# Yixin-F/DR-Using-SCV-OD

Measured on AMD Instinct MI355X. Metric: scans/sec on SemanticKITTI-seq-05-shaped input (SCV-OD dynamic-removal path, raw scans -> per-point labels + static map), higher is better.
Workload: dtype f32

## Files before the change

### dr-using-scv-od_amd/csrc/scvod_k_patchwork.inc

```
constexpr int kClsThreads = 256;
constexpr int kClsItems = 8;

__global__ __launch_bounds__(kClsThreads) void k_pw_classify(DevParams P, Arena A) {
    __shared__ int hist[kMaxPatches];
    const int s = blockIdx.y;
    const int base = A.scan_off[s];
    const int n = A.scan_off[s + 1] - base;
    const int start = blockIdx.x * (kClsThreads * kClsItems);
    if (start >= n) return;
    for (int b = threadIdx.x; b < P.n_patches; b += kClsThreads) hist[b] = 0;
    __syncthreads();
    float4 pt[kClsItems];
#pragma unroll
    for (int it = 0; it < kClsItems; ++it) {
        const int i = start + it * kClsThreads + threadIdx.x;
        pt[it] = A.pts[base + min(i, n - 1)];
    }
#pragma unroll
    for (int it = 0; it < kClsItems; ++it) {
        const int i = start + it * kClsThreads + threadIdx.x;
        if (i < n) {
            const float4 p = pt[it];
            int pid = czm_patch_of(P.czm, p.x, p.y, p.z);
            A.pid[base + i] = (int16_t)pid;
            A.zkey[base + i] = float_sort_key(p.z);
            if (pid >= 0) atomicAdd(&hist[pid], 1);
        }
    }
    __syncthreads();
    for (int b = threadIdx.x; b < P.n_patches; b += kClsThreads) {
        int c = hist[b];
        if (c) atomicAdd(&A.patch_count[s * kMaxPatches + b], c);
    }
}

__global__ __launch_bounds__(1024) void k_pw_offsets(DevParams P, Arena A) {
    __shared__ int wsum[17];
    const int s = blockIdx.x;
    int c = (threadIdx.x < (unsigned)P.n_patches) ? A.patch_count[s * kMaxPatches + threadIdx.x] : 0;
    int total;
    int ex = block_excl_scan<1024>(c, total, wsum);
    if (threadIdx.x <= (unsigned)P.n_patches) A.patch_off[s * (kMaxPatches + 1) + threadIdx.x] = ex;
}

__global__ __launch_bounds__(kClsThreads) void k_pw_scatter(DevParams P, Arena A) {
    __shared__ int hist[kMaxPatches];
    const int s = blockIdx.y;
    const int base = A.scan_off[s];
    const int n = A.scan_off[s + 1] - base;
    const int start = blockIdx.x * (kClsThreads * kClsItems);
    if (start >= n) return;
    for (int b = threadIdx.x; b < P.n_patches; b += kClsThreads) hist[b] = 0;
    __syncthreads();
    int pid[kClsItems], rank[kClsItems];
    uint32_t zk[kClsItems];
#pragma unroll
    for (int it = 0; it < kClsItems; ++it) {
        const int i = start + it * kClsThreads + threadIdx.x;
        pid[it] = (i < n) ? (int)A.pid[base + i] : -1;
        zk[it] = A.zkey[base + min(i, n - 1)];
    }
#pragma unroll
    for (int it = 0; it < kClsItems; ++it)
        rank[it] = wave_bin_rank(hist, pid[it]);
    __syncthreads();
    for (int b = threadIdx.x; b < P.n_patches; b += kClsThreads) {
        int c = hist[b];
        if (c) hist[b] = A.patch_off[s * (kMaxPatches + 1) + b] + atomicAdd(&A.patch_cursor[s * kMaxPatches + b], c);
    }
    __syncthreads();
#pragma unroll
    for (int it = 0; it < kClsItems; ++it) {
        int i = start + it * kClsThreads + threadIdx.x;
        if (i < n && pid[it] >= 0) A.keys[(size_t)base + hist[pid[it]] + rank[it]] = pack_key(zk[it], (uint32_t)i);
    }
}

constexpr int kClassXS = 32, kClassM = 40, kClassM2 = 44, kClassL = 48;
#ifndef SCVOD_FIT_COOP_CLASS
#define SCVOD_FIT_COOP_CLASS 36
#endif
constexpr int kClassFitCoop = SCVOD_FIT_COOP_CLASS;

__device__ __forceinline__ void order_range(const int32_t* off, int c_lo, int c_hi, int& lo, int& hi) {
    lo = off[c_hi];
    hi = (c_lo == 0) ? off[64] : off[c_lo - 1];
}

constexpr bool pw_sort_padfree(int cap) { return SCVOD_SORT_PADFREE == 2 || (SCVOD_SORT_PADFREE == 1 && cap >= 2048); }

template <int CAP, int THREADS, int C_LO, int C_HI, int LGE>
__global__ __launch_bounds__(THREADS)
__attribute__((amdgpu_waves_per_eu(pw_sort_padfree(CAP) ? (CAP >= 1024 ? 4 : 6) : 1, 8)))
void k_pw_sort(DevParams P, Arena A) {
    extern __shared__ __attribute__((aligned(16))) unsigned char smem[];
    int lo, hi;
    order_range(A.order_off, C_LO, C_HI, lo, hi);
    constexpr int PK = (CAP == 4096) ? 1 : 2;
    constexpr bool PADFREE = pw_sort_padfree(CAP);
    PROF_BEGIN();
    for (int w = lo + blockIdx.x; w < hi; w += gridDim.x) {
        const int4 item = A.order[w];
        const int n = item.y, base = item.z, off = item.w;
        const bool in_lds = (n <= CAP);
        unsigned long long* keys;
        if (CAP >= 4096) PROF_RESET();
        if (in_lds) {
            keys = (unsigned long long*)smem;
            int np2 = 1 << LGE;
            while (np2 < n) np2 <<= 1;
            const int nlive = sortnet::live_end(n, LGE);
            constexpr int IT = CAP / THREADS;
            const unsigned long long* gk = (const unsigned long long*)A.keys + (size_t)base + off;
            bool from_regs = false;
            if constexpr (IT == (1 << LGE) && CAP >= 4096) {
                if (np2 == CAP) {
                    from_regs = true;
                    unsigned long long tmp[IT];
                    if constexpr (PADFREE) {
                        if ((int)threadIdx.x < (nlive >> LGE)) {
#pragma unroll
                            for (int it = 0; it < IT; ++it) {
                                const int j = sortnet::start_key(it, (int)threadIdx.x, nlive, LGE);
                                tmp[it] = (j < n) ? gk[j] : kKeyPad;
                            }
                        }
                        if (CAP >= 4096) PROF_MARK(PK, 0);
                        padfree_sort_regs<THREADS, true, LGE>(tmp, keys, np2, nlive, (unsigned long long)kKeyPad);
                    } else {
#pragma unroll
                        for (int it = 0; it < IT; ++it) {
                            const int j = it * THREADS + (int)threadIdx.x;
                            tmp[it] = (j < n) ? gk[j] : kKeyPad;
                        }
                        if (CAP >= 4096) PROF_MARK(PK, 0);
                        block_bitonic_sort_pow2_regs<THREADS, true, LGE>(tmp, keys);
                    }
                }
            }
            if (!from_regs) {
                const int nfill = PADFREE ? nlive : np2;
                for (int j = threadIdx.x; j < nfill; j += THREADS) keys[sort_slot<true>(j)] = (j < n) ? gk[j] : kKeyPad;
                __syncthreads();
                if (CAP >= 4096) PROF_MARK(PK, 0);
                if constexpr (PADFREE)
                    padfree_sort<THREADS, true, LGE>(keys, np2, nlive, (unsigned long long)kKeyPad);
                else
                    block_bitonic_sort_pow2<THREADS, true, LGE>(keys, np2);
            }
            if (CAP >= 4096) PROF_MARK(PK, 1);
        } else {
            keys = (unsigned long long*)(A.keys + (size_t)base + off);
            block_bitonic_sort<THREADS, false>(keys, n);
        }
        Xyz* dst = A.sorted_xyz + (size_t)base + off;
        uint32_t* dsti = A.sorted_idx + (size_t)base + off;
        for (int j0 = threadIdx.x; j0 < n; j0 += 4 * THREADS) {
            uint32_t id[4];
            float4 q[4];
#pragma unroll
            for (int u = 0; u < 4; ++u) {
                const int j = min(j0 + u * THREADS, n - 1);
                id[u] = key_idx(keys[in_lds ? sort_slot<true>(j) : j]);
            }
#pragma unroll
            for (int u = 0; u < 4; ++u) q[u] = A.pts[base + id[u]];
#pragma unroll
            for (int u = 0; u < 4; ++u) {
                const int j = j0 + u * THREADS;
                if (j < n) {
                    Xyz o;
                    o.x = q[u].x;
                    o.y = q[u].y;
                    o.z = q[u].z;
                    dst[j] = o;
                    dsti[j] = id[u];
                }
            }
        }
        __syncthreads();
        if (CAP >= 4096) PROF_MARK(PK, 2);
    }
}

constexpr int kClassWave = 24;
__global__ __launch_bounds__(256) void k_pw_sort_wave(DevParams P, Arena A) {
    const int lane = threadIdx.x & 63;
    const int wave = threadIdx.x >> 6;
    int lo, hi;
    order_range(A.order_off, 0, kClassWave - 1, lo, hi);
    for (int w = lo + blockIdx.x * 4 + wave; w < hi; w += gridDim.x * 4) {
        const int4 item = A.order[w];
        const int n = item.y, base = item.z, off = item.w;
        unsigned long long key = (lane < n) ? A.keys[(size_t)base + off + lane] : kKeyPad;
#pragma unroll
        for (int k = 2; k <= 64; k <<= 1) {
#pragma unroll
            for (int j = k >> 1; j >= 1; j >>= 1) {
                const unsigned long long other = __shfl_xor(key, j, 64);
                const bool take_min = (((lane & k) == 0) == ((lane & j) == 0));
                unsigned long long mn = key, mx = other;
                cswap_asc(mn, mx);
                key = take_min ? mn : mx;
            }
        }
        if (lane < n) {
            const uint32_t id = key_idx(key);
            const float4 q = A.pts[base + id];
            Xyz o;
            o.x = q.x;
            o.y = q.y;
            o.z = q.z;
            A.sorted_xyz[(size_t)base + off + lane] = o;
            A.sorted_idx[(size_t)base + off + lane] = id;
        }
    }
}

__device__ __forceinline__ int pw_size_class(int n) {
    int lg = 31 - __clz(n);
    int frac = (lg >= 2) ? ((n >> (lg - 2)) & 3) : 0;
    int c = lg * 4 + frac;
    return c > 63 ? 63 : c;
}

__global__ __launch_bounds__(256) void k_pw_order_count(DevParams P, Arena A) {
    __shared__ int hist[64];
    if (threadIdx.x < 64) hist[threadIdx.x] = 0;
    __syncthreads();
    const int t = blockIdx.x * 256 + threadIdx.x;
    if (t < A.n_scans * P.n_patches) {
        const int s = t / P.n_patches, p = t - s * P.n_patches;
        const int n = A.patch_count[s * kMaxPatches + p];
        if (n <= P.czm.num_min_pts) {
            PatchRec r = {n, 0, 0, 0, 0};
            A.patch_rec[s * kMaxPatches + p] = r;
            scvod_patch_plane pl = {};
            pl.n_pts = n;
            A.planes[s * kMaxPatches + p] = pl;
        } else {
            atomicAdd(&hist[pw_size_class(n)], 1);
        }
    }
    __syncthreads();
    if (threadIdx.x < 64 && hist[threadIdx.x]) atomicAdd(&A.order_hist[threadIdx.x], hist[threadIdx.x]);
}

__global__ __launch_bounds__(64) void k_pw_order_offsets(Arena A) {
    const int c = 63 - threadIdx.x;
    const int v = A.order_hist[c];
    const int inc = wave_incl_scan(v);
    A.order_off[c] = inc - v;
    if (threadIdx.x == 63) A.order_off[64] = inc;
}

__global__ __launch_bounds__(256) void k_pw_order_scatter(DevParams P, Arena A) {
    __shared__ int hist[64];
    if (threadIdx.x < 64) hist[threadIdx.x] = 0;
    __syncthreads();
    const int t = blockIdx.x * 256 + threadIdx.x;
    int c = -1, rank = 0;
    int4 item = make_int4(0, 0, 0, 0);
    if (t < A.n_scans * P.n_patches) {
        const int s = t / P.n_patches, p = t - s * P.n_patches;
        const int n = A.patch_count[s * kMaxPatches + p];
        if (n > P.czm.num_min_pts) {
            c = pw_size_class(n);
            rank = atomicAdd(&hist[c], 1);
            item = make_int4(s * kMaxPatches + p, n, A.scan_off[s], A.patch_off[s * (kMaxPatches + 1) + p]);
        }
    }
    __syncthreads();
    if (threadIdx.x < 64 && hist[threadIdx.x])
        hist[threadIdx.x] = A.order_off[threadIdx.x] + atomicAdd(&A.order_cursor[threadIdx.x], hist[threadIdx.x]);
    __syncthreads();
    if (c >= 0) A.order[hist[c] + rank] = item;
}

__global__ __launch_bounds__(256) void k_vx_order_count(DevParams P, Arena A) {
    __shared__ int hist[64];
    if (threadIdx.x < 64) hist[threadIdx.x] = 0;
    __syncthreads();
    const int t = blockIdx.x * 256 + threadIdx.x;
    if (t < A.n_scans * P.n_buckets) {
        const int s = t / P.n_buckets, b = t - s * P.n_buckets;
        const int m = A.vb_count[s * kMaxBuckets + b];
        if (m > 0)
            atomicAdd(&hist[pw_size_class(m)], 1);
        else
            A.vb_nvox[s * kMaxBuckets + b] = 0;
    }
    __syncthreads();
    if (threadIdx.x < 64 && hist[threadIdx.x]) atomicAdd(&A.vorder_hist[threadIdx.x], hist[threadIdx.x]);
}

__global__ __launch_bounds__(64) void k_vx_order_offsets(Arena A) {
    const int c = 63 - threadIdx.x;
    const int v = A.vorder_hist[c];
    const int inc = wave_incl_scan(v);
    A.vorder_off[c] = inc - v;
    if (threadIdx.x == 63) A.vorder_off[64] = inc;
}

__global__ __launch_bounds__(256) void k_vx_order_scatter(DevParams P, Arena A) {
    __shared__ int hist[64];
    if (threadIdx.x < 64) hist[threadIdx.x] = 0;
    __syncthreads();
    const int t = blockIdx.x * 256 + threadIdx.x;
    int c = -1, rank = 0;
    int4 item = make_int4(0, 0, 0, 0);
    if (t < A.n_scans * P.n_buckets) {
        const int s = t / P.n_buckets, b = t - s * P.n_buckets;
        const int m = A.vb_count[s * kMaxBuckets + b];
        if (m > 0) {
            c = pw_size_class(m);
            rank = atomicAdd(&hist[c], 1);
            item = make_int4(s * kMaxBuckets + b, m, A.scan_off[s], A.vb_off[s * (kMaxBuckets + 1) + b]);
        }
    }
    __syncthreads();
    if (threadIdx.x < 64 && hist[threadIdx.x])
        hist[threadIdx.x] = A.vorder_off[threadIdx.x] + atomicAdd(&A.vorder_cursor[threadIdx.x], hist[threadIdx.x]);
    __syncthreads();
    if (c >= 0) A.vorder[hist[c] + rank] = item;
}

__device__ __forceinline__ float plane_res(const Xyz& q, float n0, float n1, float n2) {
    float r = q.x * n0;
    r = r + q.y * n1;
    r = r + q.z * n2;
    return r;
}

struct FitState {
    float cov[9];
    float mean0, mean1, mean2;
    float n0, n1, n2, thd;
    float sv0, sv1, sv2;
};
__device__ __forceinline__ void fit_state_init(FitState& F) {
#pragma unroll
    for (int k = 0; k < 9; ++k) F.cov[k] = 0.f;
    F.mean0 = F.mean1 = F.mean2 = 0.f;
    F.n0 = F.n1 = F.n2 = F.thd = 0.f;
    F.sv0 = F.sv1 = F.sv2 = 0.f;
}

__device__ __forceinline__ void fit_update(FitState& F, const CzmParams& cz, float a0, float a1, float a2, float a3, float a4,
                                           float a5, float a6, float a7, float a8, int m) {
    if (m != 0) {
        const float fn = (float)m;
        a0 = a0 / fn;
        a1 = a1 / fn;
        a2 = a2 / fn;
        a3 = a3 / fn;
        a4 = a4 / fn;
        a5 = a5 / fn;
        a6 = a6 / fn;
        a7 = a7 / fn;
        a8 = a8 / fn;
        F.mean0 = a6;
        F.mean1 = a7;
        F.mean2 = a8;
        F.cov[0] = a0 - a6 * a6;
        F.cov[1] = a1 - a6 * a7;
        F.cov[2] = a2 - a6 * a8;
        F.cov[4] = a3 - a7 * a7;
        F.cov[5] = a4 - a7 * a8;
        F.cov[8] = a5 - a8 * a8;
        F.cov[3] = F.cov[1];
        F.cov[6] = F.cov[2];
        F.cov[7] = F.cov[5];
    }
    Svd3 sv;
    svd3_jacobi(F.cov, sv);
    F.n0 = sv.U[2];
    F.n1 = sv.U[5];
    F.n2 = sv.U[8];
    F.sv0 = sv.sv[0];
    F.sv1 = sv.sv[1];
    F.sv2 = sv.sv[2];
    float dot = F.n0 * F.mean0;
    dot = dot + F.n1 * F.mean1;
    dot = dot + F.n2 * F.mean2;
    const float d = -dot;
    F.thd = (float)(cz.th_dist - (double)d);
}

__device__ __forceinline__ int fit_status(const DevParams& P, int zone, int ring, int concentric_idx, const FitState& F) {
    const double ground_z_vec = (double)fabs_f(F.n2);
    const double ground_z_elevation = (double)F.mean2;
    float svmin = F.sv0;
    if (F.sv1 < svmin) svmin = F.sv1;
    if (F.sv2 < svmin) svmin = F.sv2;
    const double surface_variable = (double)(svmin / (F.sv0 + F.sv1 + F.sv2));
    if (ground_z_vec < P.czm.uprightness_thr) return 2;
    if (concentric_idx < P.czm.num_rings_of_interest) {
        const int e = ring + 2 * zone;
        if (ground_z_elevation > P.czm.elevation_thr[e]) return (P.czm.flatness_thr[e] > surface_variable) ? 1 : 3;
    }
    return 1;
}

__device__ __forceinline__ void fit_finish(const DevParams& P, const Arena& A, int s, int p, int n, int zone, int ring,
                                           int concentric_idx, const FitState& F) {
    const float n0 = F.n0, n1 = F.n1, n2 = F.n2, thd = F.thd, mean0 = F.mean0, mean1 = F.mean1, mean2 = F.mean2;
    const float sv0 = F.sv0, sv1 = F.sv1, sv2 = F.sv2;
    const int status = fit_status(P, zone, ring, concentric_idx, F);
    scvod_patch_plane pl;
    pl.normal[0] = n0;
    pl.normal[1] = n1;
    pl.normal[2] = n2;
    pl.mean[0] = mean0;
    pl.mean[1] = mean1;
    pl.mean[2] = mean2;
    pl.sv[0] = sv0;
    pl.sv[1] = sv1;
    pl.sv[2] = sv2;
    pl.n_pts = n;
    pl.n_ground = 0;
    pl.status = status;
    A.planes[s * kMaxPatches + p] = pl;
    A.fit_thd[s * kMaxPatches + p] = thd;
}

__device__ __forceinline__ uint32_t triple_of_point(const DevParams& P, float x, float y, float z) {
    int32_t ri, si, ai;
    if (!idx3_fast(P.bin, P.binfast, x, y, z, &ri, &si, &ai)) {
        Apri a;
        apri_of_point(P.bin, x, y, z, 0.f, a);
        ri = a.range_idx;
        si = a.sector_idx;
        ai = a.azimuth_idx;
    }
    return (uint32_t)pack_idx3(ri, si, ai);
}

template <int GL, bool LEAN>
__device__ __forceinline__ void arrange_group(const DevParams& P, const Arena& A, const Xyz* __restrict__ sp, const uint32_t* __restrict__ si, uint32_t* seg,
                                              uint32_t* stage, int n, int n_max, int slot, bool live, int r, int gbase, float n0, float n1, float n2, float thd, int status) {
    constexpr unsigned long long FULL = (GL == 64) ? ~0ull : ((1ull << (GL & 63)) - 1ull);
    auto group_bits = [&](unsigned long long ballot) -> unsigned long long { return (ballot >> gbase) & FULL; };
    const bool rejected = (status >= 2);
    const int n_last = max(n - 1, 0);
    int n_g = 0, n_ng = 0, a_g = 0, a_ng = 0;
    Xyz q_next = sp[min(r, n_last)];
    uint32_t w_next = si[min(r, n_last)];
    const unsigned long long below = (1ull << r) - 1ull;
// ... 706 lines not shown
```

### dr-using-scv-od_amd/csrc/scvod_kernels.hip

```cpp
#include <type_traits>

#include "scvod_boxgrid.h"
#include "scvod_grid.h"
#include "scvod_sortnet.h"
#include <rocprim/device/device_radix_sort.hpp>

namespace scvod {

#ifdef SCVOD_PROFILE
__device__ unsigned long long g_prof[8][16];
#define PROF_BEGIN() unsigned long long t_prev = wall_clock64()
#define PROF_RESET()                                   \
    do {                                               \
        __syncthreads();                               \
        if (threadIdx.x == 0) t_prev = wall_clock64(); \
    } while (0)
#define PROF_MARK(k, i)                                      \
    do {                                                     \
        __syncthreads();                                     \
        if (threadIdx.x == 0) {                              \
            const unsigned long long t_now = wall_clock64(); \
            atomicAdd(&g_prof[k][i], t_now - t_prev);        \
            t_prev = t_now;                                  \
        }                                                    \
    } while (0)
#else
#define PROF_BEGIN()
#define PROF_RESET()
#define PROF_MARK(k, i)
#endif
#define CC_MARK(i) PROF_MARK(0, i)
#define CCW_MARK(i) PROF_MARK(4, i)

template <typename T>
__device__ __forceinline__ void cswap(T& x, T& y) {
    const T lo = x < y ? x : y;
    const T hi = x < y ? y : x;
    x = lo;
    y = hi;
}

template <bool PAD>
__device__ __forceinline__ int sort_slot(int i) {
    return PAD ? i + (i >> 3) : i;
}

template <int THREADS, bool PAD, typename T>
__device__ __forceinline__ void block_bitonic_sort(T* a, int n) {
#define IX(i) sort_slot<PAD>(i)
    if (n <= 1) return;
    const T INF = ~(T)0;
    int np2 = 8;
    while (np2 < n) np2 <<= 1;
    for (int g = threadIdx.x; g < (np2 >> 3); g += THREADS) {
        const int b = g << 3;
        if (b >= n) continue;
        T e[8];
#pragma unroll
        for (int m = 0; m < 8; ++m) e[m] = (b + m < n) ? a[IX(b + m)] : INF;
        cswap(e[0], e[1]); cswap(e[2], e[3]); cswap(e[4], e[5]); cswap(e[6], e[7]);
        cswap(e[0], e[2]); cswap(e[1], e[3]); cswap(e[4], e[6]); cswap(e[5], e[7]);
        cswap(e[1], e[2]); cswap(e[5], e[6]);
        cswap(e[0], e[4]); cswap(e[1], e[5]); cswap(e[2], e[6]); cswap(e[3], e[7]);
        cswap(e[2], e[4]); cswap(e[3], e[5]);
        cswap(e[1], e[2]); cswap(e[3], e[4]); cswap(e[5], e[6]);
#pragma unroll
        for (int m = 0; m < 8; ++m)
            if (b + m < n) a[IX(b + m)] = e[m];
    }
    __syncthreads();
    const int half = np2 >> 1;
    for (int k = 16; k <= np2; k <<= 1) {
        const int hk = k >> 1;
        for (int t = threadIdx.x; t < half; t += THREADS) {
            const int blk = t / hk, off = t - blk * hk;
            const int i = blk * k + off, j = blk * k + (k - 1 - off);
            if (j < n) {
                T x = a[IX(i)], y = a[IX(j)];
                if (x > y) {
                    a[IX(i)] = y;
                    a[IX(j)] = x;
                }
            }
        }
        __syncthreads();
        int j = k >> 2;
        while (j >= 1) {
            if (j >= 4) {
                const int jl = j >> 2;
                for (int t = threadIdx.x; t < (np2 >> 3); t += THREADS) {
                    const int b = (t / jl) * (jl << 3) + (t % jl);
                    if (b >= n) continue;
                    T e[8];
#pragma unroll
                    for (int m = 0; m < 8; ++m) e[m] = (b + m * jl < n) ? a[IX(b + m * jl)] : INF;
                    cswap(e[0], e[4]); cswap(e[1], e[5]); cswap(e[2], e[6]); cswap(e[3], e[7]);
                    cswap(e[0], e[2]); cswap(e[1], e[3]); cswap(e[4], e[6]); cswap(e[5], e[7]);
                    cswap(e[0], e[1]); cswap(e[2], e[3]); cswap(e[4], e[5]); cswap(e[6], e[7]);
#pragma unroll
                    for (int m = 0; m < 8; ++m)
                        if (b + m * jl < n) a[IX(b + m * jl)] = e[m];
                }
                j >>= 3;
            } else if (j == 2) {
                for (int t = threadIdx.x; t < (np2 >> 2); t += THREADS) {
                    const int b = t << 2;
                    if (b >= n) continue;
                    T e[4];
#pragma unroll
                    for (int m = 0; m < 4; ++m) e[m] = (b + m < n) ? a[IX(b + m)] : INF;
                    cswap(e[0], e[2]); cswap(e[1], e[3]);
                    cswap(e[0], e[1]); cswap(e[2], e[3]);
#pragma unroll
                    for (int m = 0; m < 4; ++m)
                        if (b + m < n) a[IX(b + m)] = e[m];
                }
                j = 0;
            } else {
                for (int t = threadIdx.x; t < half; t += THREADS) {
                    const int i = t << 1;
                    if (i + 1 < n) {
                        T x = a[IX(i)], y = a[IX(i + 1)];
                        if (x > y) {
                            a[IX(i)] = y;
                            a[IX(i + 1)] = x;
                        }
                    }
                }
                j = 0;
            }
            __syncthreads();
        }
    }
}
#undef IX

__device__ __forceinline__ int wave_bin_rank(int* hist, int bin) {
    const int lane = threadIdx.x & 63;
    int rank = 0;
    bool todo = bin >= 0;
    while (__any(todo)) {
        const int first = __ffsll((long long)__ballot(todo)) - 1;
        const int b0 = __shfl(bin, first);
        const bool mine = todo && (bin == b0);
        const unsigned long long mask = __ballot(mine);
        int old = 0;
        if (lane == first) old = atomicAdd(&hist[b0], __popcll(mask));
        old = __shfl(old, first);
        if (mine) {
            rank = old + __popcll(mask & ((1ull << lane) - 1ull));
            todo = false;
        }
    }
    return rank;
}
__device__ __forceinline__ void wave_bin_add(int* hist, int bin) {
    const int lane = threadIdx.x & 63;
    bool todo = bin >= 0;
    while (__any(todo)) {
        const int first = __ffsll((long long)__ballot(todo)) - 1;
        const int b0 = __shfl(bin, first);
        const bool mine = todo && (bin == b0);
        const unsigned long long mask = __ballot(mine);
        if (lane == first) atomicAdd(&hist[b0], __popcll(mask));
        if (mine) todo = false;
    }
}

constexpr int kKeyIdxBits = 19;
static_assert((1 << kKeyIdxBits) >= SCVOD_MAX_SCAN_POINTS, "index field of the sort keys");
constexpr unsigned long long kKeyExp = 0x3ffull << 52;
constexpr unsigned long long kKeyPad = 0x4000000000000000ull;
__device__ __forceinline__ unsigned long long pack_key(uint32_t key, uint32_t idx) {
    return kKeyExp | ((unsigned long long)key << kKeyIdxBits) | idx;
}
__device__ __forceinline__ uint32_t key_idx(unsigned long long k) { return (uint32_t)k & ((1u << kKeyIdxBits) - 1u); }
__device__ __forceinline__ uint32_t key_major(unsigned long long k) { return (uint32_t)(k >> kKeyIdxBits); }


__device__ __forceinline__ void cswap_asc(unsigned long long& x, unsigned long long& y) {
    double lo, hi;
    const double dx = __longlong_as_double((long long)x), dy = __longlong_as_double((long long)y);
    asm("v_min_f64 %0, %1, %2" : "=v"(lo) : "v"(dx), "v"(dy));
    asm("v_max_f64 %0, %1, %2" : "=v"(hi) : "v"(dx), "v"(dy));
    x = (unsigned long long)__double_as_longlong(lo);
    y = (unsigned long long)__double_as_longlong(hi);
}
__device__ __forceinline__ void cswap_asc(uint32_t& x, uint32_t& y) {
    const uint32_t lo = x < y ? x : y;
    const uint32_t hi = x < y ? y : x;
    x = lo;
    y = hi;
}

template <int LT, typename T>
__device__ __forceinline__ void reg_merge(T (&e)[1 << LT]) {
#pragma unroll
    for (int d = (1 << LT) >> 1; d >= 1; d >>= 1) {
#pragma unroll
        for (int m = 0; m < (1 << LT); ++m)
            if ((m & d) == 0) cswap_asc(e[m], e[m + d]);
    }
}

template <int THREADS, bool PAD, int LT, typename T>
__device__ __forceinline__ void bitonic_pass(T* a, int np2, int k, int r) {
    constexpr int E = 1 << LT;
    const int jl = 1 << (r - LT);
    for (int t = threadIdx.x; t < (np2 >> LT); t += THREADS) {
        const int b = ((t >> (r - LT)) << r) | (t & (jl - 1));
        const int rev = ((b & k) == 0) ? 0 : (E - 1);
        T e[E];
#pragma unroll
        for (int m = 0; m < E; ++m) e[m] = a[sort_slot<PAD>(b + (m ^ rev) * jl)];
        reg_merge<LT>(e);
#pragma unroll
        for (int m = 0; m < E; ++m) a[sort_slot<PAD>(b + (m ^ rev) * jl)] = e[m];
    }
    __syncthreads();
}

template <bool PAD, int LGE, typename T>
__device__ __forceinline__ void bitonic_run_to_lds(T (&e)[1 << LGE], T* a, int b) {
    constexpr int E = 1 << LGE;
#pragma unroll
    for (int kk = 2; kk <= E; kk <<= 1) {
#pragma unroll
        for (int d = kk >> 1; d >= 1; d >>= 1) {
#pragma unroll
            for (int m = 0; m < E; ++m)
                if ((m & d) == 0) {
                    if (kk == E || (m & kk) == 0)
                        cswap_asc(e[m], e[m + d]);
                    else
                        cswap_asc(e[m + d], e[m]);
                }
        }
    }
    const int rev = ((b & E) == 0) ? 0 : (E - 1);
#pragma unroll
    for (int m = 0; m < E; ++m) a[sort_slot<PAD>(b + (m ^ rev))] = e[m];
}

template <int THREADS, bool PAD, int LGE, typename T>
__device__ __forceinline__ void block_bitonic_merge_stages(T* a, int np2);

template <int THREADS, bool PAD, int LGE, typename T>
__device__ __forceinline__ void block_bitonic_sort_pow2(T* a, int np2) {
    constexpr int E = 1 << LGE;
    for (int g = threadIdx.x; g < (np2 >> LGE); g += THREADS) {
        const int b = g << LGE;
        T e[E];
#pragma unroll
        for (int m = 0; m < E; ++m) e[m] = a[sort_slot<PAD>(b + m)];
        bitonic_run_to_lds<PAD, LGE>(e, a, b);
    }
    __syncthreads();
    block_bitonic_merge_stages<THREADS, PAD, LGE>(a, np2);
}

template <int THREADS, bool PAD, int LGE, typename T>
__device__ __forceinline__ void block_bitonic_sort_pow2_regs(T (&e)[1 << LGE], T* a) {
    bitonic_run_to_lds<PAD, LGE>(e, a, (int)threadIdx.x << LGE);
    __syncthreads();
    block_bitonic_merge_stages<THREADS, PAD, LGE>(a, THREADS << LGE);
}

template <int THREADS, bool PAD, int LGE, typename T>
__device__ __forceinline__ void block_bitonic_merge_stages(T* a, int np2) {
    constexpr int E = 1 << LGE;
    int lgk = LGE + 1;
    for (int k = 2 * E; k <= np2; k <<= 1, ++lgk) {
        int r = lgk;
        const int first = (r % LGE) ? (r % LGE) : LGE;
        if (first == 1)
            bitonic_pass<THREADS, PAD, 1>(a, np2, k, r);
        else if (first == 2)
            bitonic_pass<THREADS, PAD, 2>(a, np2, k, r);
        else if (first == 3)
            bitonic_pass<THREADS, PAD, 3>(a, np2, k, r);
        else
            bitonic_pass<THREADS, PAD, 4>(a, np2, k, r);
        r -= first;
        while (r > 0) {
            bitonic_pass<THREADS, PAD, LGE>(a, np2, k, r);
            r -= LGE;
        }
    }
}

#ifndef SCVOD_SORT_PADFREE
#define SCVOD_SORT_PADFREE 1
#endif
#ifndef SCVOD_VOX_PADFREE
#define SCVOD_VOX_PADFREE 1
#endif
struct CxAsc {
    template <typename T>
    __device__ __forceinline__ void operator()(T& lo, T& hi) const { cswap_asc(lo, hi); }
};

template <int THREADS, bool PAD, int LT, bool MIRROR, typename T>
__device__ __forceinline__ void padfree_pass(T* a, int np2, int nlive, int r, T padv) {
    const int items = sortnet::pass_items(np2, nlive, r, LT);
    for (int t = threadIdx.x; t < items; t += THREADS) sortnet::pass_item<LT, MIRROR, PAD, T>(a, t, r, nlive, padv, CxAsc{});
    __syncthreads();
}

template <int THREADS, bool PAD, int LGE, typename T>
__device__ __forceinline__ void padfree_merge_stages(T* a, int np2, int nlive, T padv) {
    sortnet::for_each_pass<LGE>(np2, [&](int r, int lt, bool mirror) {
        if (!mirror)
            padfree_pass<THREADS, PAD, LGE, false>(a, np2, nlive, r, padv);
        else if (lt == 1)
            padfree_pass<THREADS, PAD, 1, true>(a, np2, nlive, r, padv);
        else if (lt == 2)
            padfree_pass<THREADS, PAD, 2, true>(a, np2, nlive, r, padv);
        else if (lt == 3 || LGE == 3)
            padfree_pass<THREADS, PAD, 3, true>(a, np2, nlive, r, padv);
        else if constexpr (LGE >= 4)
            padfree_pass<THREADS, PAD, 4, true>(a, np2, nlive, r, padv);
    });
}

template <int THREADS, bool PAD, int LGE, typename T>
__device__ __forceinline__ void padfree_sort(T* a, int np2, int nlive, T padv) {
    constexpr int E = 1 << LGE;
    for (int g = threadIdx.x; g < (nlive >> LGE); g += THREADS) {
        T e[E];
#pragma unroll
        for (int m = 0; m < E; ++m) e[m] = a[sort_slot<PAD>((g << LGE) + m)];
        sortnet::run_store<LGE, PAD>(e, a, g, CxAsc{});
    }
    __syncthreads();
    padfree_merge_stages<THREADS, PAD, LGE>(a, np2, nlive, padv);
}

template <int THREADS, bool PAD, int LGE, typename T>
__device__ __forceinline__ void padfree_sort_regs(T (&e)[1 << LGE], T* a, int np2, int nlive, T padv) {
    if ((int)threadIdx.x < (nlive >> LGE)) sortnet::run_store<LGE, PAD>(e, a, (int)threadIdx.x, CxAsc{});
    __syncthreads();
    padfree_merge_stages<THREADS, PAD, LGE>(a, np2, nlive, padv);
}

#include "scvod_k_patchwork.inc"
#include "scvod_k_voxelgrid.inc"
#include "scvod_k_voxels.inc"
#include "scvod_k_cluster.inc"
#include "scvod_k_merge.inc"
#include "scvod_k_rgrow.inc"
#include "scvod_k_calib.inc"
#include "scvod_k_probe_nn.inc"
#define TH_BEGIN(name) \
    if (th) th(tu, name, 1)
#define TH_END(name) \
    if (th) th(tu, name, 0)

#ifndef SCVOD_SORT_LGE
#define SCVOD_SORT_LGE 4
#endif
constexpr int kLGE = SCVOD_SORT_LGE;
constexpr int kTS = (kLGE == 4) ? 1 : 2;
#ifndef SCVOD_VOX_LGE
#define SCVOD_VOX_LGE 3
#endif
constexpr int kLGEv = SCVOD_VOX_LGE, kTSv = (kLGEv == 4) ? 1 : 2;
constexpr int kPersistCUs = 256;
constexpr int kSortCapS = 1024, kSortThreadsS = 64;
constexpr int kSortCapL = 8192, kSortThreadsL = 512;
constexpr int kSortCapXL = 16384, kClassXL = 52;
constexpr size_t sort_lds_bytes(int cap) { return (size_t)(cap + cap / 8) * 8; }
constexpr int kVoxCapS = 1024, kVoxThreadsS = 64;
constexpr int kVoxCapL = 8192, kVoxThreadsL = 512;

template <int CAP, int THREADS, int C_LO, int C_HI, int LGE, typename KT, bool DESC>
static void launch_vx_tier(const DevParams& P, const Arena& A, hipStream_t st, int per_cu_network) {
    if constexpr (vx_bucket_counting(CAP, sizeof(KT), 0, DESC)) {
        if (P.vb_shift == kVxCountShift) {
            constexpr size_t lds = vox_lds_bytes(CAP, sizeof(KT), DESC, true);
            constexpr int per_cu_counting = vx_count_per_cu(CAP, DESC);
            static_assert(per_cu_counting > 0 && per_cu_counting * lds <= 160 * 1024, "workgroups per CU of a counting tier");
            if (CAP >= 4096)
                hipFuncSetAttribute((const void*)k_vx_bucket<CAP, THREADS, C_LO, C_HI, LGE, 0, KT, DESC, true>, hipFuncAttributeMaxDynamicSharedMemorySize, (int)lds);
            hipLaunchKernelGGL((k_vx_bucket<CAP, THREADS, C_LO, C_HI, LGE, 0, KT, DESC, true>), dim3(kPersistCUs * per_cu_counting), dim3(THREADS), lds, st, P, A);
            return;
        }
    }
    constexpr size_t lds = vox_lds_bytes(CAP, sizeof(KT), DESC);
    if (CAP >= 4096)
        hipFuncSetAttribute((const void*)k_vx_bucket<CAP, THREADS, C_LO, C_HI, LGE, 0, KT, DESC, false>, hipFuncAttributeMaxDynamicSharedMemorySize, (int)lds);
    hipLaunchKernelGGL((k_vx_bucket<CAP, THREADS, C_LO, C_HI, LGE, 0, KT, DESC, false>), dim3(kPersistCUs * per_cu_network), dim3(THREADS), lds, st, P, A);
}

void launch_process(const DevParams& P, const Arena& A, hipStream_t st, int do_patchwork, int apply_filter,
                    int do_voxels, TimerHook th, void* tu, int lean_voxels, int lean_emit) {
    const int B = A.n_scans;
    if (B <= 0) return;
    if (do_patchwork == 1) {
        hipMemsetAsync(A.patch_count, 0, sizeof(int32_t) * (size_t)B * kMaxPatches, st);
        hipMemsetAsync(A.patch_cursor, 0, sizeof(int32_t) * (size_t)B * kMaxPatches, st);
        dim3 gcls((A.max_scan_pts + kClsThreads * kClsItems - 1) / (kClsThreads * kClsItems), B);
        TH_BEGIN("pw_classify");
        hipLaunchKernelGGL(k_pw_classify, gcls, dim3(kClsThreads), 0, st, P, A);
        TH_END("pw_classify");
        TH_BEGIN("pw_offsets");
        hipLaunchKernelGGL(k_pw_offsets, dim3(B), dim3(1024), 0, st, P, A);
        TH_END("pw_offsets");
        TH_BEGIN("pw_scatter");
        hipLaunchKernelGGL(k_pw_scatter, gcls, dim3(kClsThreads), 0, st, P, A);
        TH_END("pw_scatter");
        hipMemsetAsync(A.order_hist, 0, sizeof(int32_t) * 64, st);
        hipMemsetAsync(A.order_cursor, 0, sizeof(int32_t) * 64, st);
        const int n_all = B * P.n_patches;
        TH_BEGIN("pw_order");
        hipLaunchKernelGGL(k_pw_order_count, dim3((n_all + 255) / 256), dim3(256), 0, st, P, A);
        hipLaunchKernelGGL(k_pw_order_offsets, dim3(1), dim3(64), 0, st, A);
        hipLaunchKernelGGL(k_pw_order_scatter, dim3((n_all + 255) / 256), dim3(256), 0, st, P, A);
        TH_END("pw_order");
        hipFuncSetAttribute((const void*)k_pw_sort<kSortCapXL, 1024, kClassXL, 63, 4>, hipFuncAttributeMaxDynamicSharedMemorySize,
                            (int)sort_lds_bytes(kSortCapXL));
        hipFuncSetAttribute((const void*)k_pw_sort<kSortCapL, kSortThreadsL * kTS, kClassL, kClassXL - 1, kLGE>,
                            hipFuncAttributeMaxDynamicSharedMemorySize, (int)sort_lds_bytes(kSortCapL));
        TH_BEGIN("pw_sort_8192");
        hipLaunchKernelGGL((k_pw_sort<kSortCapXL, 1024, kClassXL, 63, 4>), dim3(kPersistCUs), dim3(1024), sort_lds_bytes(kSortCapXL), st, P, A);
        hipLaunchKernelGGL((k_pw_sort<kSortCapL, kSortThreadsL * kTS, kClassL, kClassXL - 1, kLGE>), dim3(kPersistCUs * 2),
                           dim3(kSortThreadsL * kTS), sort_lds_bytes(kSortCapL), st, P, A);
        TH_END("pw_sort_8192");
        TH_BEGIN("pw_sort_4096");
        hipLaunchKernelGGL((k_pw_sort<4096, 256 * kTS, kClassM2, kClassL - 1, kLGE>), dim3(kPersistCUs * 4), dim3(256 * kTS),
                           sort_lds_bytes(4096), st, P, A);
        TH_END("pw_sort_4096");
        TH_BEGIN("pw_sort_2048");
        hipLaunchKernelGGL((k_pw_sort<2048, 128 * kTS, kClassM, kClassM2 - 1, kLGE>), dim3(kPersistCUs * 8), dim3(128 * kTS),
                           sort_lds_bytes(2048), st, P, A);
        TH_END("pw_sort_2048");
        TH_BEGIN("pw_sort_1024");
        hipLaunchKernelGGL((k_pw_sort<kSortCapS, kSortThreadsS * kTS, kClassXS, kClassM - 1, kLGE>), dim3(kPersistCUs * 16),
                           dim3(kSortThreadsS * kTS), sort_lds_bytes(kSortCapS), st, P, A);
        TH_END("pw_sort_1024");
        TH_BEGIN("pw_sort_256");
        hipLaunchKernelGGL((k_pw_sort<256, 64, kClassWave, kClassXS - 1, 3>), dim3(kPersistCUs * 32), dim3(64),
                           sort_lds_bytes(256), st, P, A);
        TH_END("pw_sort_256");
        TH_BEGIN("pw_sort_wave");
        hipLaunchKernelGGL(k_pw_sort_wave, dim3(kPersistCUs * 8), dim3(256), 0, st, P, A);
        TH_END("pw_sort_wave");
        const int coop_class = (B <= 8) ? kClassWave : kClassFitCoop;
        const int coop_min = 1 << (coop_class / 4);
        TH_BEGIN("pw_fit_large");
        const dim3 gfit((int)(A.total_pts / coop_min / (B <= 8 ? 1 : 4)) + 1);
        if (B <= 8) {
            if (lean_emit)
                hipLaunchKernelGGL((k_pw_fit_coop<64, true>), gfit, dim3(64), 0, st, P, A, coop_class);
            else
                hipLaunchKernelGGL((k_pw_fit_coop<64, false>), gfit, dim3(64), 0, st, P, A, coop_class);
        } else {
            if (lean_emit)
                hipLaunchKernelGGL((k_pw_fit_coop<16, true>), gfit, dim3(64), 0, st, P, A, coop_class);
            else
                hipLaunchKernelGGL((k_pw_fit_coop<16, false>), gfit, dim3(64), 0, st, P, A, coop_class);
        }
        TH_END("pw_fit_large");
        TH_BEGIN("pw_fit");
        hipLaunchKernelGGL(k_pw_fit, dim3((n_all + 63) / 64), dim3(64), 0, st, P, A, coop_class);
        TH_END("pw_fit");
        TH_BEGIN("pw_arrange");
        if (lean_emit) {
            if (coop_class > kClassWave) hipLaunchKernelGGL((k_pw_arrange<64, true>), dim3(kPersistCUs * 8), dim3(256), 0, st, P, A, kClassWave, coop_class - 1);
            hipLaunchKernelGGL((k_pw_arrange<16, true>), dim3(kPersistCUs * 4), dim3(256), 0, st, P, A, 0, kClassWave - 1);
        } else {
            if (coop_class > kClassWave) hipLaunchKernelGGL((k_pw_arrange<64, false>), dim3(kPersistCUs * 8), dim3(256), 0, st, P, A, kClassWave, coop_class - 1);
            hipLaunchKernelGGL((k_pw_arrange<16, false>), dim3(kPersistCUs * 4), dim3(256), 0, st, P, A, 0, kClassWave - 1);
        }
        TH_END("pw_arrange");
        TH_BEGIN("emit_offsets");
        hipLaunchKernelGGL(k_emit_offsets, dim3(B), dim3(1024), 0, st, P, A);
        TH_END("emit_offsets");
        TH_BEGIN("emit");
        if (lean_emit)
            hipLaunchKernelGGL(k_emit<true>, dim3(kPersistCUs * 8), dim3(kEmitThreads), 0, st, P, A);
        else
            hipLaunchKernelGGL(k_emit<false>, dim3(kPersistCUs * 8), dim3(kEmitThreads), 0, st, P, A);
        TH_END("emit");
    } else if (do_patchwork == 0) {
        TH_BEGIN("bin_direct");
        hipLaunchKernelGGL(k_bin_direct, dim3(B), dim3(1024), 0, st, P, A, apply_filter);
        TH_END("bin_direct");
    }
    if (do_voxels) {
        if (do_patchwork == 2) {
            hipMemsetAsync(A.scan_irr, 0, sizeof(int32_t) * (size_t)B, st);
            hipMemsetAsync(A.irr_list, 0xff, sizeof(int32_t) * (size_t)B * (kIrrListCap + 1), st);
            hipLaunchKernelGGL(k_apri_split, dim3((A.max_scan_pts + 2047) / 2048, B), dim3(256), 0, st, A);
        }
        TH_BEGIN("vx_partition");
        hipLaunchKernelGGL(k_vx_partition, dim3(B), dim3(1024), 0, st, P, A);
        TH_END("vx_partition");
        dim3 gb(P.n_buckets, B);
        hipMemsetAsync(A.vorder_hist, 0, sizeof(int32_t) * 64, st);
        hipMemsetAsync(A.vorder_cursor, 0, sizeof(int32_t) * 64, st);
        const int nb_all = B * P.n_buckets;
        TH_BEGIN("vx_order");
        hipLaunchKernelGGL(k_vx_order_count, dim3((nb_all + 255) / 256), dim3(256), 0, st, P, A);
        hipLaunchKernelGGL(k_vx_order_offsets, dim3(1), dim3(64), 0, st, A);
        hipLaunchKernelGGL(k_vx_order_scatter, dim3((nb_all + 255) / 256), dim3(256), 0, st, P, A);
        TH_END("vx_order");
        if (do_patchwork == 3) {
            hipFuncSetAttribute((const void*)k_vx_bucket<kVoxCapL, kVoxThreadsL * kTSv, kClassL, 63, kLGEv, 1>,
                                hipFuncAttributeMaxDynamicSharedMemorySize, (int)vox_lds_bytes(kVoxCapL));
            hipFuncSetAttribute((const void*)k_vx_bucket<4096, 256 * kTSv, kClassM2, kClassL - 1, kLGEv, 1>,
                                hipFuncAttributeMaxDynamicSharedMemorySize, (int)vox_lds_bytes(4096));
            hipLaunchKernelGGL((k_vx_bucket<kVoxCapL, kVoxThreadsL * kTSv, kClassL, 63, kLGEv, 1>), dim3(kPersistCUs), dim3(kVoxThreadsL * kTSv),
                               vox_lds_bytes(kVoxCapL), st, P, A);
            hipLaunchKernelGGL((k_vx_bucket<4096, 256 * kTSv, kClassM2, kClassL - 1, kLGEv, 1>), dim3(kPersistCUs * 2), dim3(256 * kTSv),
                               vox_lds_bytes(4096), st, P, A);
            hipLaunchKernelGGL((k_vx_bucket<2048, 128 * kTSv, kClassM, kClassM2 - 1, kLGEv, 1>), dim3(kPersistCUs * 4), dim3(128 * kTSv),
                               vox_lds_bytes(2048), st, P, A);
            hipLaunchKernelGGL((k_vx_bucket<kVoxCapS, kVoxThreadsS * kTSv, kClassXS, kClassM - 1, kLGEv, 1>), dim3(kPersistCUs * 8),
                               dim3(kVoxThreadsS * kTSv), vox_lds_bytes(kVoxCapS), st, P, A);
            hipLaunchKernelGGL((k_vx_bucket<256, 64, 0, kClassXS - 1, 3, 1>), dim3(kPersistCUs * 32), dim3(64), vox_lds_bytes(256), st,
                               P, A);
            hipLaunchKernelGGL(k_vx_final_offsets, dim3(B), dim3(1024), 0, st, P, A);
            return;
        }
        auto bucket_tiers = [&](auto kt, auto desc) {
            using KT = decltype(kt);
            constexpr size_t KS = sizeof(KT);
            constexpr bool DESC = decltype(desc)::value;
            constexpr int kMore = (KS == 4 && SCVOD_VOX_K32_LDS) ? (DESC ? 3 : SCVOD_VOX_LEAN_MORE) : 2;
            TH_BEGIN("vx_bucket_8192");
            launch_vx_tier<kVoxCapL, kVoxThreadsL * kTSv, kClassL, 63, kLGEv, KT, DESC>(P, A, st, 1);
            TH_END("vx_bucket_8192");
            TH_BEGIN("vx_bucket_4096");
            launch_vx_tier<4096, 256 * kTSv, kClassM2, kClassL - 1, kLGEv, KT, DESC>(P, A, st, kMore);
            TH_END("vx_bucket_4096");
            TH_BEGIN("vx_bucket_2048");
            launch_vx_tier<2048, 128 * kTSv, kClassM, kClassM2 - 1, kLGEv, KT, DESC>(P, A, st, kMore * 2);
            TH_END("vx_bucket_2048");
            TH_BEGIN("vx_bucket_1024");
            launch_vx_tier<kVoxCapS, kVoxThreadsS * kTSv, kClassXS, kClassM - 1, kLGEv, KT, DESC>(P, A, st, DESC ? 8 : SCVOD_VOX_LEAN_S);
            TH_END("vx_bucket_1024");
            TH_BEGIN("vx_bucket_256");
            launch_vx_tier<256, 64, 0, kClassXS - 1, 3, KT, DESC>(P, A, st, 32);
            TH_END("vx_bucket_256");
        };
        if (A.vx_k32) {
            if (lean_voxels)
                bucket_tiers((uint32_t)0, std::false_type{});
            else
                bucket_tiers((uint32_t)0, std::true_type{});
        } else {
            if (lean_voxels)
                bucket_tiers((unsigned long long)0, std::false_type{});
            else
                bucket_tiers((unsigned long long)0, std::true_type{});
        }
        TH_BEGIN("vx_final_offsets");
        hipLaunchKernelGGL(k_vx_final_offsets, dim3(B), dim3(1024), 0, st, P, A);
        TH_END("vx_final_offsets");
        TH_BEGIN("vx_final");
        if (lean_voxels)
            hipLaunchKernelGGL(k_vx_final<false>, dim3((P.n_buckets + 3) / 4, B), dim3(256), 0, st, P, A);
        else
            hipLaunchKernelGGL(k_vx_final<true>, dim3((P.n_buckets + 3) / 4, B), dim3(256), 0, st, P, A);
        TH_END("vx_final");
    }
}

void launch_vox_descriptors(const Arena& A, int s0, int n_scans, hipStream_t st, TimerHook th, void* tu) {
    if (n_scans <= 0 || A.max_scan_pts <= 0) return;
    TH_BEGIN("vx_descriptors");
    hipLaunchKernelGGL(k_vx_descriptors, dim3((A.max_scan_pts + 4095) / 4096, n_scans), dim3(256), 0, st, A, s0);
    TH_END("vx_descriptors");
}

void launch_apri_intensity(const Arena& A, hipStream_t st, TimerHook th, void* tu) {
    if (A.n_scans <= 0 || A.max_scan_pts <= 0) return;
    TH_BEGIN("emit_intensity");
    hipLaunchKernelGGL(k_apri_intensity, dim3((A.max_scan_pts + 2047) / 2048, A.n_scans), dim3(256), 0, st, A);
    TH_END("emit_intensity");
}

void launch_emit_lists(const Arena& A, hipStream_t st, TimerHook th, void* tu) {
    if (A.n_scans <= 0 || A.max_scan_pts <= 0) return;
    TH_BEGIN("emit_lists");
    hipLaunchKernelGGL(k_emit_lists, dim3(kPersistCUs * 8), dim3(kEmitThreads), 0, st, A);
    TH_END("emit_lists");
}

void launch_apri_expand(const DevParams& P, const Arena& A, int s0, int n_scans, int max_pts, hipStream_t st) {
    if (n_scans <= 0 || max_pts <= 0) return;
    hipLaunchKernelGGL(k_apri_expand, dim3((max_pts + 1023) / 1024, n_scans), dim3(256), 0, st, P, A, s0);
}

void launch_voxelgrid_keys(const Arena& A, const VgJob& J, hipStream_t st) {
    const int B = A.n_scans;
    if (B <= 0) return;
    hipMemsetAsync(A.vg_range, 0, sizeof(int32_t), st);
    hipLaunchKernelGGL(k_vg_minmax, dim3(B), dim3(1024), 0, st, A, J);
    if (A.max_scan_pts > 0)
        hipLaunchKernelGGL(k_vg_keys, dim3((A.max_scan_pts + 2047) / 2048, B), dim3(256), 0, st, A, J);
}
void launch_voxelgrid_lut(const Arena& A, hipStream_t st) {
    if (A.n_scans <= 0 || A.max_scan_pts <= 0) return;
    hipFuncSetAttribute((const void*)k_vg_lut, hipFuncAttributeMaxDynamicSharedMemorySize, kVgLutBins * (int)sizeof(int));
    hipLaunchKernelGGL(k_vg_lut, dim3(A.n_scans), dim3(1024), kVgLutBins * sizeof(int), st, A, (int32_t*)A.vb_lut_shift);
}
void launch_voxelgrid_gather(const DevParams& P, const Arena& A, const VgJob& J, long long out_capacity, hipStream_t st) {
    if (A.n_scans <= 0 || A.max_scan_pts <= 0) return;
    hipLaunchKernelGGL(k_vg_outoff, dim3(1), dim3(1024), 0, st, A);
    hipLaunchKernelGGL(k_vg_final, dim3(P.n_buckets, A.n_scans), dim3(256), 0, st, A, J, out_capacity);
}

void launch_cls(const Arena& A, int s, size_t scan_base, int n_points, hipStream_t st) {
    if (n_points <= 0) return;
    hipMemsetAsync(A.cls + scan_base, SCVOD_CLS_DROPPED, (size_t)n_points, st);
    hipLaunchKernelGGL(k_cls_from_lists, dim3((n_points + 2047) / 2048), dim3(256), 0, st, A, s);
}

void launch_cluster(const DevParams& P, const Arena& A0, int from_apri, hipStream_t st, TimerHook th, void* tu) {
    Arena A = A0;
    hipMemsetAsync(A.cc_stats, 0, 8 * sizeof(int32_t), st);
    const int B = A.n_scans;
    if (B <= 0 || A.max_scan_pts <= 0) return;
    A.cc_help_blocks = A.cc_help_blocks_wanted > 0 ? 1 : 0;
    hipMemsetAsync(A.cc_again, 0, sizeof(int32_t), st);
    hipMemsetAsync(A.cc_help, 0, kCcHelpWords * sizeof(int32_t), st);
    hipFuncSetAttribute((const void*)k_cc_scan, hipFuncAttributeMaxDynamicSharedMemorySize, (int)kCcLdsBytes);
    hipFuncSetAttribute((const void*)k_cc_exact, hipFuncAttributeMaxDynamicSharedMemorySize, (int)kCcLdsBytes);
    TH_BEGIN("cc_scan");
    hipLaunchKernelGGL(k_cc_order, dim3(1), dim3(1024), 0, st, A);
    hipLaunchKernelGGL(k_cc_scan, dim3(B), dim3(kCcThreads), kCcLdsBytes, st, P, A, from_apri);
    TH_END("cc_scan");
    TH_BEGIN("cc_exact");
    hipLaunchKernelGGL(k_cc_exact, dim3(kCcExactBlocks), dim3(kCcThreads), kCcLdsBytes, st, P, A, from_apri);
    TH_END("cc_exact");
}

size_t merge_lds_bytes(const DevParams& P, int max_scan_pts) {
    return 4 * ((size_t)P.bin.range_num * P.bin.azimuth_num + 1 + ((size_t)max_scan_pts + 31) / 32);
}

void launch_merge(const DevParams& P, const Arena& A, const MergeJob& M, int from_apri, hipStream_t st, TimerHook th, void* tu) {
    hipMemsetAsync(M.stats, 0, 8 * sizeof(int32_t), st);
    const int B = A.n_scans;
// ... 197 lines not shown
```

Baseline: 97570.

## Replace bitonic merge stages with merge-path merging in large patch sorts

Adds a merge-path sort for the LDS-resident patch key sort at capacities 4096-8192. After the per-thread 16-element sorting network, each level merges pairs of sorted runs: every thread binary-searches its split point and then serially merges 16 outputs. This replaces the log^2 bitonic/padfree merge passes with log levels of linear merges, cutting compare-exchange passes and barriers. The cost is binary-search LDS reads and data-dependent branching, which can cause bank conflicts and divergence.

Result: faster. 99230, median of 6 (+1.7%).

```diff
diff --git a/dr-using-scv-od_amd/csrc/scvod_k_patchwork.inc b/dr-using-scv-od_amd/csrc/scvod_k_patchwork.inc
--- a/dr-using-scv-od_amd/csrc/scvod_k_patchwork.inc
+++ b/dr-using-scv-od_amd/csrc/scvod_k_patchwork.inc
@@ -88,6 +88,9 @@
 }
 
 constexpr bool pw_sort_padfree(int cap) { return SCVOD_SORT_PADFREE == 2 || (SCVOD_SORT_PADFREE == 1 && cap >= 2048); }
+constexpr bool pw_sort_merge(int cap) {
+    return pw_sort_padfree(cap) && cap >= 2048 && cap <= 8192 && (SCVOD_SORT_MERGE == 2 || (SCVOD_SORT_MERGE == 1 && cap >= 4096));
+}
 
 template <int CAP, int THREADS, int C_LO, int C_HI, int LGE>
 __global__ __launch_bounds__(THREADS)
@@ -98,6 +101,7 @@
     order_range(A.order_off, C_LO, C_HI, lo, hi);
     constexpr int PK = (CAP == 4096) ? 1 : 2;
     constexpr bool PADFREE = pw_sort_padfree(CAP);
+    constexpr bool MERGE = pw_sort_merge(CAP) && LGE == 4 && (THREADS << LGE) == CAP;
     PROF_BEGIN();
     for (int w = lo + blockIdx.x; w < hi; w += gridDim.x) {
         const int4 item = A.order[w];
@@ -126,7 +130,10 @@
                             }
                         }
                         if (CAP >= 4096) PROF_MARK(PK, 0);
-                        padfree_sort_regs<THREADS, true, LGE>(tmp, keys, np2, nlive, (unsigned long long)kKeyPad);
+                        if constexpr (MERGE)
+                            mergepath_sort_regs<THREADS, true, LGE, SCVOD_SORT_MERGE_RUN>(tmp, keys, np2, nlive, (unsigned long long)kKeyPad);
+                        else
+                            padfree_sort_regs<THREADS, true, LGE>(tmp, keys, np2, nlive, (unsigned long long)kKeyPad);
                     } else {
 #pragma unroll
                         for (int it = 0; it < IT; ++it) {
@@ -143,7 +150,9 @@
                 for (int j = threadIdx.x; j < nfill; j += THREADS) keys[sort_slot<true>(j)] = (j < n) ? gk[j] : kKeyPad;
                 __syncthreads();
                 if (CAP >= 4096) PROF_MARK(PK, 0);
-                if constexpr (PADFREE)
+                if constexpr (MERGE)
+                    mergepath_sort<THREADS, true, LGE, SCVOD_SORT_MERGE_RUN>(keys, np2, nlive, (unsigned long long)kKeyPad);
+                else if constexpr (PADFREE)
                     padfree_sort<THREADS, true, LGE>(keys, np2, nlive, (unsigned long long)kKeyPad);
                 else
                     block_bitonic_sort_pow2<THREADS, true, LGE>(keys, np2);
diff --git a/dr-using-scv-od_amd/csrc/scvod_kernels.hip b/dr-using-scv-od_amd/csrc/scvod_kernels.hip
--- a/dr-using-scv-od_amd/csrc/scvod_kernels.hip
+++ b/dr-using-scv-od_amd/csrc/scvod_kernels.hip
@@ -3,6 +3,7 @@
 #include "scvod_boxgrid.h"
 #include "scvod_grid.h"
 #include "scvod_sortnet.h"
+#include "scvod_mergepath.h"
 #include <rocprim/device/device_radix_sort.hpp>
 
 namespace scvod {
@@ -341,6 +342,60 @@
     if ((int)threadIdx.x < (nlive >> LGE)) sortnet::run_store<LGE, PAD>(e, a, (int)threadIdx.x, CxAsc{});
     __syncthreads();
     padfree_merge_stages<THREADS, PAD, LGE>(a, np2, nlive, padv);
+}
+
+#ifndef SCVOD_SORT_MERGE
+#define SCVOD_SORT_MERGE 1
+#endif
+#ifndef SCVOD_SORT_MERGE_RUN
+#define SCVOD_SORT_MERGE_RUN 16
+#endif
+static_assert(SCVOD_SORT_MERGE_RUN >= 16 && SCVOD_SORT_MERGE_RUN <= 1024 && (SCVOD_SORT_MERGE_RUN & (SCVOD_SORT_MERGE_RUN - 1)) == 0,
+              "SCVOD_SORT_MERGE_RUN");
+
+template <int THREADS, bool PAD, int LGE, int RUN, typename T>
+__device__ __forceinline__ void mergepath_levels(T* a, int np2, int nlive, T padv) {
+    static_assert(RUN >= (1 << LGE), "the merge levels start from whole register runs");
+    if constexpr (RUN > (1 << LGE)) {
+        sortnet::for_each_pass<LGE>(np2 < RUN ? np2 : RUN, [&](int r, int lt, bool mirror) {
+            if (!mirror)
+                padfree_pass<THREADS, PAD, LGE, false>(a, np2, nlive, r, padv);
+            else if (lt == 1)
+                padfree_pass<THREADS, PAD, 1, true>(a, np2, nlive, r, padv);
+            else if (lt == 2)
+                padfree_pass<THREADS, PAD, 2, true>(a, np2, nlive, r, padv);
+            else if (lt == 3 || LGE == 3)
+                padfree_pass<THREADS, PAD, 3, true>(a, np2, nlive, r, padv);
+            else if constexpr (LGE >= 4)
+                padfree_pass<THREADS, PAD, 4, true>(a, np2, nlive, r, padv);
+        });
+    }
+    for (int L = RUN; L < nlive; L <<= 1) {
+        T out[1 << LGE];
+        const bool mine = mergepath::merge_window<LGE, PAD, T>(a, (int)threadIdx.x, L, nlive, out, ~(T)0);
+        __syncthreads();
+        if (mine) mergepath::store_window<LGE, PAD, T>(a, (int)threadIdx.x, out);
+        __syncthreads();
+    }
+}
+
+template <int THREADS, bool PAD, int LGE, int RUN, typename T>
+__device__ __forceinline__ void mergepath_sort(T* a, int np2, int nlive, T padv) {
+    constexpr int E = 1 << LGE;
+    for (int g = threadIdx.x; g < (nlive >> LGE); g += THREADS) {
+        T e[E];
+#pragma unroll
+        for (int m = 0; m < E; ++m) e[m] = a[sort_slot<PAD>((g << LGE) + m)];
+        sortnet::run_store<LGE, PAD>(e, a, g, CxAsc{});
+    }
+    __syncthreads();
+    mergepath_levels<THREADS, PAD, LGE, RUN>(a, np2, nlive, padv);
+}
+template <int THREADS, bool PAD, int LGE, int RUN, typename T>
+__device__ __forceinline__ void mergepath_sort_regs(T (&e)[1 << LGE], T* a, int np2, int nlive, T padv) {
+    if ((int)threadIdx.x < (nlive >> LGE)) sortnet::run_store<LGE, PAD>(e, a, (int)threadIdx.x, CxAsc{});
+    __syncthreads();
+    mergepath_levels<THREADS, PAD, LGE, RUN>(a, np2, nlive, padv);
 }
 
 #include "scvod_k_patchwork.inc"
diff --git a/dr-using-scv-od_amd/csrc/scvod_mergepath.h b/dr-using-scv-od_amd/csrc/scvod_mergepath.h
--- /dev/null
+++ b/dr-using-scv-od_amd/csrc/scvod_mergepath.h
@@ -0,0 +1,76 @@
+#pragma once
+
+#include "scvod_sortnet.h"
+
+namespace mergepath {
+
+struct Pair {
+    int a0, a1;
+    int b0, b1;
+    int d;
+};
+SORTNET_HD constexpr int imin(int x, int y) { return x < y ? x : y; }
+SORTNET_HD constexpr int imax(int x, int y) { return x > y ? x : y; }
+
+SORTNET_HD constexpr Pair pair_of(int p, int L, int nlive) {
+    const int a0 = p & ~(2 * L - 1);
+    const int b0 = imin(a0 + L, nlive);
+    return Pair{a0, b0, b0, imin(a0 + 2 * L, nlive), p - a0};
+}
+
+SORTNET_HD constexpr int levels(int run0, int nlive) {
+    int c = 0;
+    for (int L = run0; L < nlive; L <<= 1) ++c;
+    return c;
+}
+
+template <bool PAD, typename T, typename Arr>
+SORTNET_HD int split(Arr a, const Pair& q) {
+    int lo = imax(0, q.d - (q.b1 - q.b0)), hi = imin(q.d, q.a1 - q.a0);
+    while (lo < hi) {
+        const int mid = (lo + hi) >> 1;
+        const T ka = a[sortnet::slot(PAD, q.a0 + mid)];
+        const T kb = a[sortnet::slot(PAD, q.b0 + q.d - 1 - mid)];
+        if (kb < ka)
+            hi = mid;
+        else
+            lo = mid + 1;
+    }
+    return lo;
+}
+
+template <int LGE, bool PAD, typename T, typename Arr>
+SORTNET_HD bool merge_window(Arr a, int t, int L, int nlive, T (&out)[1 << LGE], T sent, int* ia = nullptr) {
+    constexpr int E = 1 << LGE;
+    const int p = t << LGE;
+    if (p >= nlive) return false;
+    const Pair q = pair_of(p, L, nlive);
+    if (q.b0 == q.b1) return false;
+    const int i = split<PAD, T>(a, q);
+    if (ia) *ia = i;
+    int xa = q.a0 + i, xb = q.b0 + (q.d - i);
+    T ha = sent, hb = sent;
+    if (xa < q.a1) ha = a[sortnet::slot(PAD, xa)];
+    if (xb < q.b1) hb = a[sortnet::slot(PAD, xb)];
+#pragma unroll
+    for (int s = 0; s < E; ++s) {
+        const bool take_a = !(hb < ha);
+        out[s] = take_a ? ha : hb;
+        if (s + 1 < E) {
+            if (take_a) ++xa; else ++xb;
+            const int x = take_a ? xa : xb;
+            T v = sent;
+            if (x < (take_a ? q.a1 : q.b1)) v = a[sortnet::slot(PAD, x)];
+            if (take_a) ha = v; else hb = v;
+        }
+    }
+    return true;
+}
+
+template <int LGE, bool PAD, typename T, typename Arr>
+SORTNET_HD void store_window(Arr a, int t, const T (&out)[1 << LGE]) {
+#pragma unroll
+    for (int m = 0; m < (1 << LGE); ++m) a[sortnet::slot(PAD, (t << LGE) + m)] = out[m];
+}
+
+}
```
